# longfish/Multigrid-FEANet

Measured on AMD Instinct MI355X. Metric: DoF-updates/sec per V-cycle (fp64) + achieved HBM GB/s, 4097² Poisson, higher is better.
Workload: dtype f64; 1 GPU; 4097x4097 poisson f64 V-cycle, L=12, V(1,1) (MultiGrid.Step semantics), batch 1 per GPU; mode=single, batch=1, levels=12, parallelism=single GPU

## Files before the change

multigrid-feanet_amd/csrc/framed_ops.hip:

```cpp
#include "framed_strip.h"

namespace fea {

__device__ __forceinline__ int lin_block(int rev) {
  const int bid = xcd_remap(blockIdx.x, gridDim.x);
  return rev ? (int)gridDim.x - 1 - bid : bid;
}

__device__ __forceinline__ TaskId decode_task_lin(int nstrips, int ntr, int rev = 0) {
  const int per = ntr * nstrips;
  const int wpb = (per + kWaves - 1) / kWaves;
  const int bid = lin_block(rev);
  TaskId id;
  id.b = bid / wpb;
  const int w = (bid - id.b * wpb) * kWaves + __builtin_amdgcn_readfirstlane((int)(threadIdx.x >> 6));
  id.t = w / nstrips;
  id.s = w - id.t * nstrips;
  id.valid = w < per;
  return id;
}

template <typename T>
__device__ __forceinline__ void norm_partial(const MgArgs<T>& g, double ssq) {
  ssq = wave_sum(ssq);
// ... 1640 lines not shown
      if (y - 4 >= r0) iter(y - 4, std::integral_constant<int, 2 % D>{});
  }
}

template <typename T, bool MULTI>
__global__ __launch_bounds__(256) void k_mg_prolong2(MgArgs<T> g) {
  __shared__ T tab[MULTI ? FEA_MAX_PATTERNS * kTabStride : 1];
  __shared__ T ptb[MULTI ? FEA_MAX_PATTERNS * kTabStride : 1];
  if constexpr (MULTI) {
    load_tables<T>(tab, g.ktab, g.omd, g.ntab, ptb, g.ptab, g.nptab);
    __syncthreads();
  }
  const TaskId id = decode_task_lin(g.nstrips, g.ntr);
  if (!id.valid) return;
  if constexpr (sizeof(T) == 8) {
    if (id.t & 1) {
      prolong2_task<T, MULTI, true>(g, id, tab, ptb);
      return;
    }
  }
  prolong2_task<T, MULTI, false>(g, id, tab, ptb);
}

template <int SECOND, typename X>
__device__ __forceinline__ X& pick(X& a, X& b) {
  if constexpr (SECOND) return b;
  else return a;
}

#ifndef FEA_JOIN_AHEAD
#define FEA_JOIN_AHEAD 2
#endif
static_assert(FEA_JOIN_AHEAD == 2 || FEA_JOIN_AHEAD == 4, "join prefetch ring of 2 or 4 rows");
#ifndef FEA_JOIN_UNROLL
#define FEA_JOIN_UNROLL 4
#endif
constexpr int kJoinUnroll = FEA_JOIN_UNROLL;
static_assert(kJoinUnroll % FEA_JOIN_AHEAD == 0 && kJoinUnroll % 2 == 0, "join unroll: a multiple of the ring");
template <int N, typename Fn, int... I>
__device__ __forceinline__ void unroll_steps_(Fn&& fn, std::integer_sequence<int, I...>) {
  (fn(std::integral_constant<int, I>{}), ...);
}
template <int N, typename Fn>
__device__ __forceinline__ void unroll_steps(Fn&& fn) {
  unroll_steps_<N>(fn, std::make_integer_sequence<int, N>{});
}
// ... 850 lines not shown
template <typename T>
static int prolong2(const T* fc, const T* ec2, const T* f, T* out, const uint8_t* pid, const uint8_t* pidc,
                    const uint8_t* pidc2, const T* ktab, const T* omd, int ntab, const T* ptab, int nptab, T w1, int B,
                    int H, int W, int ld, long long bs, int ldc, long long bsc, int ldc2, long long bsc2,
                    void* stream) {
  if (!fc || !ec2 || !f || !out || !omd || !ptab || B <= 0 || !layout_ok<T>(H, W, ld, bs)) return FEA_EINVAL;
  if (!coarse_ok<T>(H, W, ldc, bsc) || !coarse_ok<T>((H + 1) / 2, (W + 1) / 2, ldc2, bsc2)) return FEA_EINVAL;
  const bool multi = ntab > 1;
  if (!tab_ok(ktab, ntab, pid) || (multi && (!pidc || !pidc2)) || !xtab_ok(nptab, ntab)) return FEA_EINVAL;
  MgArgs<T> g = mg_args<T>(H, W, ld, bs, B);
  g.ec = fc; g.ec2 = ec2; g.f = f; g.out = out; g.pid = pid; g.pidc = pidc; g.pidc2 = pidc2; g.ktab = ktab;
  g.omd = omd; g.ntab = ntab; g.ptab = ptab; g.nptab = nptab; g.w = w1;
  mg_coarse(g, ldc, bsc);
  mg_coarse2(g, ldc2, bsc2);
  g.nstrips = div_up(W - 2, Ovl4<T>::S);
  const int u2 = pick_rb(B, g.nstrips, H - 2) / 2;
  g.rb = 2 * balanced_units(B, g.nstrips, (H - 1) / 2, 2, 4, u2, u2);
  g.ntr = div_up(H - 2, g.rb);
  const dim3 grid = mg_grid_lin(B, g.ntr, g.nstrips);
  hipStream_t s = (hipStream_t)stream;
  if (multi) k_mg_prolong2<T, true><<<grid, 256, 0, s>>>(g);
  else k_mg_prolong2<T, false><<<grid, 256, 0, s>>>(g);
  return launch_status();
}

#define FEA_MG_API(SUF, T)                                                                                           \
  extern "C" int fea_mg_pack_##SUF(const T* src, T* dst, const T* geo, long long geo_bs, const T* bc, long long bc_bs, \
                                   int B, int H, int W, int ld, long long bs, void* stream) {                         \
    return mg_pack<T>(src, dst, geo, geo_bs, bc, bc_bs, B, H, W, ld, bs, stream);                                     \
  }                                                                                                                  \
  extern "C" int fea_mg_unpack_##SUF(const T* src, T* dst, int B, int H, int W, int ld, long long bs, void* stream) { \
    return mg_unpack<T>(src, dst, B, H, W, ld, bs, stream);                                                          \
  }                                                                                                                  \
  extern "C" int fea_mg_sweep_##SUF(const T* u, const T* f, T* out, const uint8_t* pid, const T* ktab, const T* omd,   \
                                    int ntab, int B, int H, int W, int ld, long long bs, void* stream) {              \
    return mg_sweep<T>(u, f, out, pid, ktab, omd, ntab, B, H, W, ld, bs, stream);                                    \
  }                                                                                                                  \
  extern "C" int fea_mg_residual_restrict_##SUF(const T* u, const T* f, T* v_out, T* fc, const uint8_t* pid,          \
                                                const T* ktab, const T* omd, int ntab, const T* rtab, int nrtab,      \
                                                T w0, int B, int H, int W, int ld, long long bs, int ldc,            \
                                                long long bsc, void* stream) {                                       \
    return mg_residual_restrict<T>(u, f, v_out, fc, pid, ktab, omd, ntab, rtab, nrtab, w0, B, H, W, ld, bs, ldc, bsc,  \
                                   stream);                                                                          \
  }                                                                                                                  \
  extern "C" int fea_mg_zero_restrict_send_##SUF(const T* f, T* fc, const uint8_t* pid, const T* ktab, const T* omd,   \
                                                 int ntab, const T* rtab, int nrtab, T w0, int B, int H, int W,       \
// ... 72 lines not shown
```

multigrid-feanet_amd/csrc/mid_ops.hip:

```cpp
#include "fea_common.h"

namespace fea {

constexpr int kMidThreads = 1024;
constexpr int kMidMaxK = 4;
constexpr int kMidLdsBytes = 160 * 1024 - 2048;
constexpr int kMS = 10;

#ifdef FEA_MID_TRACE
__device__ long long g_mid_trace[4096];
#define FEA_MID_MARK(slot) \
  if (threadIdx.x == 0) g_mid_trace[slot] = (long long)__builtin_amdgcn_s_memrealtime()
#define FEA_MID_SYNC(ph)                                                                   \
  do {                                                                                     \
    __syncthreads();                                                                       \
    if (blockIdx.x == 0 && threadIdx.x == 0) g_mid_trace[2048 + (ph)] = (long long)__builtin_amdgcn_s_memrealtime(); \
  } while (0)
#define FEA_MID_WAVE_MARK(slot)                                                              \
  if (blockIdx.x == 0 && (threadIdx.x & 63) == 0)                                            \
  g_mid_trace[3072 + (slot) * 16 + (threadIdx.x >> 6)] = (long long)__builtin_amdgcn_s_memrealtime()
#else
#define FEA_MID_MARK(slot)
#define FEA_MID_SYNC(ph) __syncthreads()
#define FEA_MID_WAVE_MARK(slot)
// ... 590 lines not shown
    const int Y0 = wv * per, Y1 = min(U0.nr, Y0 + per);
    constexpr int CH = MULTI ? 2 : 4;
    for (int s0 = Y0; s0 < Y1; s0 += CH) {
      const int n = min(CH, Y1 - s0);
      if constexpr (CH == 4) {
        if (n == 4) chunk(std::integral_constant<int, 4>{}, s0, s0 + 4);
        else if (n == 3) chunk(std::integral_constant<int, 3>{}, s0, s0 + 3);
        else if (n == 2) chunk(std::integral_constant<int, 2>{}, s0, s0 + 2);
        else chunk(std::integral_constant<int, 1>{}, s0, s0 + 1);
      } else {
        if (n == 2) chunk(std::integral_constant<int, 2>{}, s0, s0 + 2);
        else chunk(std::integral_constant<int, 1>{}, s0, s0 + 1);
      }
    }
    if (j > 0) FEA_MID_SYNC(1 + (k - 1 - j));
  }
  FEA_MID_MARK(2 * blockIdx.x + 1);
}

}

using namespace fea;

template <typename T>
static int mid_fill(MidArgs<T>& a, int k, int B, int H, int W, int TR, int TC) {
  if (k < 1 || k > kMidMaxK || B <= 0 || B > 65535 || TR < 1 || TC < 1) return FEA_EINVAL;
  a.k = k;
  for (int j = 0; j <= k; ++j) {
    if (H < 3 || W < 3 || (j < k && (!(H & 1) || !(W & 1)))) return FEA_EINVAL;
    a.H[j] = H;
    a.W[j] = W;
    if (fea_mg_layout(H, W, (int)sizeof(T), &a.ld[j], &a.bs[j]) != 0) return FEA_EINVAL;
    H = (H + 1) / 2;
    W = (W + 1) / 2;
  }
  a.TR = TR;
  a.TC = TC;
  return 0;
}

template <typename T, bool MULTI, typename Kern>
static void mid_launch(Kern k1, Kern k2, Kern k3, Kern k4, int k, dim3 grid, void* stream, const MidArgs<T>& a) {
  Kern kern = k == 1 ? k1 : k == 2 ? k2 : k == 3 ? k3 : k4;
  hipLaunchKernelGGL(kern, grid, dim3(kMidThreads), 0, (hipStream_t)stream, a);
}

template <typename T, bool GATHER>
static int mid_down(const T* const* f, const uint8_t* const* pid, int k, int B, int H, int W, const T* ktab,
                    const T* omd, int ntab, const T* rtab, int nrtab, T w0, int TR, int TC, const T* gsrc, int Pr,
                    int Pc, int gcr, int gcc, void* stream) {
  MidArgs<T> a = {};
  if (!f || !omd || !rtab || !tab_ok(ktab, ntab, pid) || !xtab_ok(nrtab, ntab)) return FEA_EINVAL;
  if (GATHER && (!gsrc || Pr < 1 || Pc < 1 || gcr < 1 || gcc < 1 || H - 1 != Pr * gcr || W - 1 != Pc * gcc))
    return FEA_EINVAL;
  const bool multi = ntab > 1;
  if (mid_fill<T>(a, k, B, H, W, TR, TC)) return FEA_EINVAL;
  if (mid_down_lds(k, TR, TC, (int)sizeof(T), multi) > kMidLdsBytes) return FEA_EINVAL;
  for (int j = 0; j <= k; ++j) {
    if (!f[j] || (multi && j < k && !pid[j])) return FEA_EINVAL;
    a.f[j] = f[j];
    a.fo[j] = const_cast<T*>(f[j]);
    a.pid[j] = multi && j < k ? pid[j] : nullptr;
  }
  a.ktab = ktab; a.omd = omd; a.xtab = rtab; a.w = w0; a.ntab = ntab; a.nx = nrtab;
  if (GATHER) {
    a.gsrc = gsrc; a.gB = B; a.gPc = Pc; a.gcr = gcr; a.gcc = gcc;
  }
  a.ntr = (a.H[k] - 2 + TR - 1) / TR;
  a.ntc = (a.W[k] - 2 + TC - 1) / TC;
  const dim3 grid(B * a.ntr * a.ntc);
  if (multi) mid_launch<T, true>(k_mg_mid_down<T, true, 1, GATHER>, k_mg_mid_down<T, true, 2, GATHER>,
                                 k_mg_mid_down<T, true, 3, GATHER>, k_mg_mid_down<T, true, 4, GATHER>, k, grid,
                                 stream, a);
  else mid_launch<T, false>(k_mg_mid_down<T, false, 1, GATHER>, k_mg_mid_down<T, false, 2, GATHER>,
                            k_mg_mid_down<T, false, 3, GATHER>, k_mg_mid_down<T, false, 4, GATHER>, k, grid,
                            stream, a);
  return launch_status();
}

template <typename T>
static int mid_up(const T* const* f, const T* e, T* out, const uint8_t* const* pid, int k, int B, int H, int W,
                  const T* ktab, const T* omd, int ntab, const T* ptab, int nptab, T w1, int TR, int TC,
                  void* stream) {
  MidArgs<T> a = {};
  if (!f || !e || !out || !omd || !ptab || !tab_ok(ktab, ntab, pid) || !xtab_ok(nptab, ntab)) return FEA_EINVAL;
  const bool multi = ntab > 1;
  if (mid_fill<T>(a, k, B, H, W, TR, TC)) return FEA_EINVAL;
  if (mid_up_lds(k, TR, TC, (int)sizeof(T), multi) > kMidLdsBytes) return FEA_EINVAL;
  for (int j = 0; j <= k; ++j) {
    if ((j < k && (!f[j] || f[j] == out)) || (multi && !pid[j])) return FEA_EINVAL;
    a.f[j] = j < k ? f[j] : nullptr;
    a.pid[j] = multi ? pid[j] : nullptr;
  }
  if (e == out) return FEA_EINVAL;
  a.e = e; a.out = out;
  a.ktab = ktab; a.omd = omd; a.xtab = ptab; a.w = w1; a.ntab = ntab; a.nx = nptab;
  a.ntr = (a.H[0] - 2 + TR - 1) / TR;
  a.ntc = (a.W[0] - 2 + TC - 1) / TC;
  const dim3 grid(B * a.ntr * a.ntc);
  if (multi) mid_launch<T, true>(k_mg_mid_up<T, true, 1>, k_mg_mid_up<T, true, 2>, k_mg_mid_up<T, true, 3>,
                                 k_mg_mid_up<T, true, 4>, k, grid, stream, a);
  else mid_launch<T, false>(k_mg_mid_up<T, false, 1>, k_mg_mid_up<T, false, 2>, k_mg_mid_up<T, false, 3>,
                            k_mg_mid_up<T, false, 4>, k, grid, stream, a);
  return launch_status();
}

#define FEA_MID_API(SUF, T)                                                                                        \
  extern "C" int fea_mg_mid_down_##SUF(const T* const* f, const uint8_t* const* pid, int k, int B, int H, int W,    \
                                       const T* ktab, const T* omd, int ntab, const T* rtab, int nrtab, T w0,       \
// ... 31 lines not shown
```

multigrid-feanet_amd/feanet_amd/schedule.py:

```python


def _other(b):
    return "b" if b == "a" else "a"


OMDF = "omdf"


def vcycle_schedule(L, nu1=1, nu2=1, compat=None, start="a", tail_from=None, fuse=True, top_zero=False,
                    recompute=True):
    if tail_from is not None and not (1 <= tail_from <= L - 1):
        raise ValueError("vcycle_schedule: tail_from must be in [1, L-1]")
    if L < 1 or nu1 < 0 or nu2 < 0:
        raise ValueError("vcycle_schedule: need L >= 1, nu1, nu2 >= 0")
    if compat not in (None, "mm_interface_q2"):
        raise ValueError(f"vcycle_schedule: unknown compat mode {compat!r}")
    steps = []
    cur = ["zero"] * L
    cur[0] = "zero" if top_zero else start

    def sweep(l, zero=False):
        dst = "a" if (zero or cur[l] == "zero") else _other(cur[l])
        steps.append(("sweep", l, None if (zero or cur[l] == "zero") else cur[l], dst))
        cur[l] = dst
# ... 174 lines not shown
            k = len(run)
            while k > 0:
                if k >= 2 and can_pair(run[k - 1][1]):
                    paired.append(("prolong_sweep2", run[k - 1][1], run[k - 2][3], run[k - 1][4]))
                    k -= 2
                else:
                    paired.append(run[k - 1])
                    k -= 1
            paired.reverse()
        else:
            k = 0
            while k < len(run):
                if k + 1 < len(run) and can_pair(run[k + 1][1]):
                    paired.append(("prolong_sweep2", run[k + 1][1], run[k][3], run[k + 1][4]))
                    k += 2
                else:
                    paired.append(run[k])
                    k += 1
        out.extend(paired)
        i = j
    return out


def group_mid(steps, pick_down, pick_up):
    out = []
    i = 0
    n = len(steps)
    while i < n:
        st = steps[i]
        if st[0] == "resid_restrict" and st[2] is None and st[3] is None:
            j = i
            while (j + 1 < n and steps[j + 1][0] == "resid_restrict" and steps[j + 1][2] is None
                   and steps[j + 1][3] is None and steps[j + 1][1] == steps[j][1] + 1):
                j += 1
            run = steps[i:j + 1]
            groups = {a: (k, T) for a, k, T in pick_down([s_[1] for s_ in run])}
            m = 0
            while m < len(run):
                l = run[m][1]
                if l in groups:
                    k, T = groups[l]
                    out.append(("mid_down", l, k, T))
                    m += k
                else:
                    out.append(run[m])
                    m += 1
# ... 44 lines not shown
```

multigrid-feanet_amd/feanet_amd/solver.py:

```python
import itertools
import math
import time
import weakref

import numpy as np
import torch

from . import _lib, mesh_setup as ms, ops
from .graphs import GraphCache
from .schedule import (OMDF, _other, extend_tail, group_hmid, group_mid, hjac_schedule, pair_prolongations, pair_restrictions,
                       vcycle_schedule)


_SOLVERS = weakref.WeakValueDictionary()
_HANDLES = itertools.count(1)


def first_sweep_raw(launches, f0, raw):
    for i, rec in enumerate(launches):
        try:
            _lib.arg(rec, "u_raw")
        except TypeError:
            continue
        if _lib.arg(rec, "f") == f0:
            return launches[:i] + [_lib.replace(rec, u_raw=raw)] + launches[i + 1:]
    return None


def solver_by_handle(h):
    s = _SOLVERS.get(int(h))
    if s is None:
        raise RuntimeError(f"feanet: no live MultigridSolver with handle {h}")
    return s
# ... 36 lines not shown
    def view(self, t):
        off = 128 // t.element_size() - 1
        return t[:self.B * self.bs].view(self.B, self.H + 2, self.ld)[:, 1:self.H + 1, off:off + self.W]

    def pid_view(self):
        return self.pid[:(self.H + 2) * self.ld].view(self.H + 2, self.ld)[1:self.H + 1, self.off:self.off + self.W]

    def geom(self):
        return (self.B, self.H, self.W, self.ld, self.bs)

    def geom_kw(self):
        return dict(B=self.B, H=self.H, W=self.W, ld=self.ld, bstride=self.bs)


class MultigridSolver:

    MID_NODES = 20000
    MID_NODES_DOWN = None
    MID_NODES_UP = None
    MID_MIN_TILES = 200
    MID_MAX_REDUNDANCY = 3.0
    HMID_NODES = 300000
    HMID_MIN_TILES = 64
    TAIL_MAX_N = 65
    TAIL_EXT = True
    TAIL_EXT_MIN_BATCH = 64

    def __init__(self, n, levels=None, problem="poisson", dtype=torch.float64, device=None, batch=1,
                 omega=2.0 / 3.0, size=2.0, prop=(1, 20), shape=0, R=None, P=None, w=(1.0, 1.0),
                 nu1=1, nu2=1, compat=None, graph=True, coarse_tail=True, fuse=True, rows=None, zero_start=False,
                 smoother="jac", hnet=None, join_cycles=True, mid=True, pair_levels=True, pid_maps=None):
        m = n if rows is None else int(rows)
        if rows is None and (n < 2 or (n & (n - 1)) != 0):
            raise ValueError(f"MultigridSolver: n={n} must be a power of two >= 2")
        if m < 2 or n < 2:
            raise ValueError(f"MultigridSolver: need >= 2 intervals each way (got {m} x {n})")
        if dtype not in (torch.float32, torch.float64):
            raise TypeError("MultigridSolver: dtype must be torch.float32 or torch.float64")
        self.device = torch.device(device if device is not None else "cuda")
        ops.require_hip(torch.empty(0, device=self.device), "solver device")
        self.n, self.m = n, m
        if levels is None:
            L = 1
            while (n % (1 << L) == 0 and m % (1 << L) == 0 and (n >> L) >= 2 and (m >> L) >= 2):
                L += 1
            self.L = L if rows is not None else int(math.log2(n))
# ... 235 lines not shown
            w = [float(x) for x in (w.detach().cpu().tolist() if torch.is_tensor(w) else w)]
            if (w[0], w[1]) != self.w:
                self.w = (w[0], w[1])
                self._plans.clear()
                self._graphs.clear()

    def _ptr(self, lvl, name):
        if name == OMDF:
            return None
        return self.levels[lvl].buf(name).data_ptr()

    def _build(self, start):
        if self.smoother == "hjac":
            steps, end = hjac_schedule(self.L, self.nu1, self.nu2, "zero" if self.zero_start else start,
                                       tail_from=self.hjac_tail_from, fuse=self.fuse)
            if self.mid and self.fuse:
                steps = group_hmid(steps, self._pick_hmid())
        else:
            steps, end = vcycle_schedule(self.L, self.nu1, self.nu2, self.compat, start, self.tail_from, self.fuse,
                                         top_zero=self.zero_start)
            if self.mid:
                steps = group_mid(steps, lambda lv: self._pick_mid(lv, False), lambda lv: self._pick_mid(lv, True))
            if self.pair_levels:
                ok = lambda l: l + 2 < self.L and self.levels[l + 2].H >= 3 and self.levels[l + 2].W >= 3
                steps = pair_prolongations(pair_restrictions(steps, ok), ok)
            if self._tail_ext_ok():
                steps = extend_tail(steps)
        return [self.bind_step(st) for st in steps], end

    def _tail_ext_ok(self):
        t = self.tail_from
        return (self.TAIL_EXT and t is not None and self.B >= self.TAIL_EXT_MIN_BATCH and self.ntab == 1
                and self.nu1 == 1 and self.nu2 == 1 and self.compat is None and self.levels[t - 1].W <= 129 and self.levels[t - 1].H <= 129)

    def _mid_tile(self, up, a, k):
        esz = self.levels[0].esz
        multi = self.ntab > 1
        tl = self.levels[a if up else a + k]
        top = self.levels[a]
        best = None
        for T in ((128, 64, 32, 16, 8) if up else (32, 16, 8, 4, 2)):
            if _lib.mid_lds_bytes(up, k, T, T, esz, multi) <= 0:
                continue
            tiles = self.B * -(-(tl.H - 2) // T) * -(-(tl.W - 2) // T)
            if not up:
                reg = (T << k) + 3 * ((1 << k) - 1)
                if reg * reg * tiles > self.MID_MAX_REDUNDANCY * self.B * top.H * top.W:
                    continue
            best = T
            if tiles >= self.MID_MIN_TILES:
                return T
# ... 84 lines not shown

        def fs(a, n):
            return _lib.PtrArray([lv[j].f.data_ptr() for j in range(a, a + n)])

        def tail(t):
            return dict(Ht=lv[t].H, Wt=lv[t].W, nlev=self.L - t, ld_t=lv[t].ld, bs_t=lv[t].bs,
                        pid_levels=None if self.tail_pid is None else self.tail_pid.data_ptr(),
                        ktab=self.ktab.data_ptr(), omd=self.omd.data_ptr(), ntab=self.ntab, rtab=self.rtab.data_ptr(),
                        ptab=self.ptab.data_ptr(), w0=self.w[0], w1=self.w[1], nu1=self.nu1, nu2=self.nu2, B=lv[t].B)

        kind, l = st[0], st[1]
        f = lv[l].f.data_ptr()
        if kind == "sweep":
            return launch("mg_sweep", u=ptr(l, st[2]), f=f, out=ptr(l, st[3]), **sten(pid(l)), **geom(l))
        if kind == "hsweep":
            return launch("mg_hsweep", u=ptr(l, st[2]), u_raw=None, f=f, out=ptr(l, st[3]), **sten(pid(l)),
                          **self._hnet(), **geom(l))
        if kind == "resid_restrict":
            return launch("mg_residual_restrict", u=ptr(l, st[2]), f=f, v_out=ptr(l, st[3]), fc=lv[l + 1].f.data_ptr(),
                          **sten(pid(l)), **rest(), **geom(l), **cp(l))
        if kind == "resid_restrict2":
            return launch("mg_zero_restrict2", f=f, fc=lv[l + 1].f.data_ptr(), fc2=lv[l + 2].f.data_ptr(),
                          pidc=pid(l + 1), **sten(pid(l)), **rest(), **geom(l), **cp(l), **cp2(l))
        if kind == "sweep_restrict":
            return launch("mg_sweep_restrict", u=ptr(l, st[2]), f=f, u_out=ptr(l, st[3]), fc=lv[l + 1].f.data_ptr(),
                          **sten(pid(l)), **rest(), **geom(l), **cp(l), norm_ws=None, norm_hist=None, norm_cnt=None)
        if kind == "prolong_sweep":
            return launch("mg_prolong_sweep", u=ptr(l, st[2]), ec=ptr(l + 1, st[3]), f=f, out=ptr(l, st[4]),
                          pidc=pid(l + 1), **sten(pid(l)), **prol(), **geom(l), **cp(l))
        if kind == "prolong_sweep2":
            return launch("mg_prolong2", fc=lv[l + 1].f.data_ptr(), ec2=ptr(l + 2, st[2]), f=f, out=ptr(l, st[3]),
                          pidc=pid(l + 1), pidc2=pid(l + 2), **sten(pid(l)), **prol(), **geom(l), **cp(l), **cp2(l))
        if kind == "prolong_add":
            return launch("mg_prolong_add", u=ptr(l, st[2]), ec=ptr(l + 1, st[3]), out=ptr(l, st[4]), pidc=pid(l + 1),
                          **prol(), **geom(l), **cp(l))
        if kind == "mid_down":
            a, k, T = st[1], st[2], st[3]
            TR, TC = T if isinstance(T, tuple) else (T, T)
            return launch("mg_mid_down", f=fs(a, k + 1), k=k, B=self.B, H=lv[a].H, W=lv[a].W,
                          **sten(pids(a, k + 1)), **rest(), TR=TR, TC=TC)
        if kind == "mid_up":
            a, k, csrc, dst, T = st[1:6]
            TR, TC = T if isinstance(T, tuple) else (T, T)
            return launch("mg_mid_up", f=fs(a, k), e=ptr(a + k, csrc), out=ptr(a, dst), k=k, B=self.B, H=lv[a].H,
                          W=lv[a].W, **sten(pids(a, k + 1)), **prol(), TR=TR, TC=TC)
        if kind == "coarse_tail":
# ... 424 lines not shown
```

Before: 129.0 billion DoF-updates/s.

## Fuse three coarse levels into single strip kernels for restriction and prolongation

Adds strip-based kernels that process three multigrid levels in one launch. One fuses zero-start residual and restriction over three levels, the other fuses prolongation with a Jacobi sweep across three levels. A schedule pass rewrites the steps just above the coarse tail into these kernels, with only the prolongation variant switched on by default. The aim is fewer launches and fewer round trips of intermediate coarse grids through HBM on the small upper-mid levels, at the cost of redundant halo work, higher register pressure and limited parallelism.

```diff
diff --git a/multigrid-feanet_amd/csrc/framed_ops.hip b/multigrid-feanet_amd/csrc/framed_ops.hip
--- a/multigrid-feanet_amd/csrc/framed_ops.hip
+++ b/multigrid-feanet_amd/csrc/framed_ops.hip
@@ -1686,6 +1686,521 @@
   prolong2_task<T, MULTI, false>(g, id, tab, ptb);
 }
 
+template <typename T>
+struct Mg3Args {
+  MgArgs<T> g;
+  T* out3;
+  const T* ec3;
+  int Hc3, Wc3, ldc3;
+  long long bsc3;
+};
+
+template <int SH, typename T>
+__device__ __forceinline__ T shrz(T x) {
+#pragma unroll
+  for (int k = 0; k < SH; ++k) x = shr1z(x);
+  return x;
+}
+template <int SH, typename T>
+__device__ __forceinline__ T shlz(T x) {
+#pragma unroll
+  for (int k = 0; k < SH; ++k) x = shl1z(x);
+  return x;
+}
+template <typename T, int N, int SH>
+__device__ __forceinline__ Row<T, N> own_row_sh(const T (&x)[N]) {
+  Row<T, N> w;
+#pragma unroll
+  for (int k = 0; k < N; ++k) w.a[k + 1] = x[k];
+  w.a[0] = shrz<SH>(x[N - 1]);
+  w.a[N + 1] = shlz<SH>(x[0]);
+  return w;
+}
+
+template <typename T, int N, int SH>
+struct RStage {
+  static constexpr int B0 = N == 1 ? 0 : 1;
+  Row<T, N> Va{}, Vb{}, Vc{};
+  Row<T, N> Ro{}, Re{};
+  T fp[N] = {};
+
+  template <bool ODD>
+  __device__ __forceinline__ T push(const T (&o)[N], bool rin, const bool (&jin)[N], const T (&ks)[9],
+                                    const T (&rs)[9], T om, T w0) {
+    T x[N];
+#pragma unroll
+    for (int q = 0; q < N; ++q) x[q] = (rin && jin[q]) ? om * o[q] : T(0);
+    Va = Vb;
+    Vb = Vc;
+    Vc = own_row_sh<T, N, SH>(x);
+    const PRow<N> np{};
+    T r[N];
+#pragma unroll
+    for (int q = 0; q < N; ++q) r[q] = fp[q] - kapply<T, N, false>(Va, Vb, Vc, np, np, np, q, ks, nullptr);
+    const Row<T, N> R = own_row_sh<T, N, SH>(r);
+    T out = T(0);
+    if constexpr (!ODD) {
+      const int zp[1] = {0};
+      const T acc = restrict9<T, false>(rs, nullptr, Ro.a, Re.a, R.a, B0, zp, zp, zp, 0);
+      out = w0 * acc;
+      Ro = R;
+    } else {
+      Re = R;
+    }
+#pragma unroll
+    for (int q = 0; q < N; ++q) fp[q] = o[q];
+    return out;
+  }
+};
+
+template <typename T>
+struct OvlZ3 {
+  static constexpr int V = Frame<T>::VEC;
+  static constexpr int Q = V / 2;
+  static constexpr int SH3 = Q == 1 ? 2 : 1;
+  static constexpr int LN = 2 * SH3;
+  static constexpr int L1 = 1, H1 = 62;
+  static constexpr int L2 = L1 + (Q == 1 ? 2 : 1), H2 = H1 - 2;
+  static constexpr int L3 = L2 + 2 * SH3, H3 = H2 - 2 * SH3;
+  static constexpr int I0 = L3;
+  static constexpr int NC = (H3 - I0) / LN + 1;
+  static constexpr int S = 8 * NC;
+  static_assert(I0 - SH3 >= L2 && I0 - (Q == 1 ? 3 : 1) >= L1 && I0 + LN * (NC - 1) <= H3, "owned lanes are exact");
+  static_assert(V * I0 + V - 1 - 8 <= Frame<T>::OFF, "the left halo fits the frame");
+};
+
+template <typename T>
+__global__ __launch_bounds__(256) void k_mg_zero_restrict3(Mg3Args<T> a) {
+  using F = Frame<T>;
+  using O = OvlZ3<T>;
+  constexpr int V = F::VEC;
+  constexpr int Q = O::Q;
+  const MgArgs<T>& g = a.g;
+  const TaskId id = decode_task_lin(g.nstrips, g.ntr);
+  if (!id.valid) return;
+  const int lane = lane_id();
+  const int H = g.H, W = g.W, Hc = g.Hc, Wc = g.Wc, Hc2 = g.Hc2, Wc2 = g.Wc2, Hc3 = a.Hc3, Wc3 = a.Wc3;
+  const int Nlo = id.s * O::NC + 1, Nhi = Nlo + O::NC;
+  const int Mlo = 2 * Nlo - 1, Mhi = 2 * Nhi - 1;
+  const int Jlo = 2 * Mlo - 1, Jhi = 2 * Mhi - 1;
+  const int cs = 8 * Nlo - (V - 1) - V * O::I0;
+  const int cl = cs + V * lane;
+  const int J0 = (cl + 1) / 2;
+  const int M0 = Q == 1 ? (J0 >> 1) : ((J0 + 1) >> 1);
+  const int N0 = M0 >> 1;
+  const bool has2 = Q == 1 ? !(J0 & 1) : true;
+  const bool has3 = has2 && !(M0 & 1);
+  const int K0 = 1 + id.t * (g.rb / 8);
+  const int K1 = min(K0 + g.rb / 8, Hc3 - 1);
+  const bool last = K1 == Hc3 - 1;
+  const int R2lo = 2 * K0 - 1, R2hi = last ? Hc2 - 1 : 2 * K1 - 1;
+  const int R1lo = 2 * R2lo - 1, R1hi = last ? Hc - 1 : 2 * R2hi - 1;
+  T ks[9], rs[9];
+#pragma unroll
+  for (int d = 0; d < 9; ++d) {
+    ks[d] = g.ktab[d];
+    rs[d] = g.rtab[d];
+  }
+  const T om = g.omd[0];
+  const T w0 = g.w;
+  bool cin[V], jin[Q], st1[Q];
+#pragma unroll
+  for (int k = 0; k < V; ++k) cin[k] = cl + k >= 1 && cl + k <= W - 2;
+#pragma unroll
+  for (int q = 0; q < Q; ++q) {
+    jin[q] = J0 + q >= 1 && J0 + q <= Wc - 2;
+    st1[q] = J0 + q >= Jlo && J0 + q < Jhi && J0 + q <= Wc - 2;
+  }
+  const bool min2[1] = {M0 >= 1 && M0 <= Wc2 - 2};
+  const bool st2 = has2 && M0 >= Mlo && M0 < Mhi && M0 <= Wc2 - 2;
+  const bool st3 = has3 && N0 >= Nlo && N0 < Nhi && N0 <= Wc3 - 2;
+  const T* __restrict__ fb = g.f + (long long)id.b * g.bs + F::OFF + cs;
+  T* __restrict__ cb = g.out + (long long)id.b * g.bsc + F::OFF + J0;
+  T* __restrict__ cb2 = g.out2 + (long long)id.b * g.bsc2 + F::OFF + M0;
+  T* __restrict__ cb3 = a.out3 + (long long)id.b * a.bsc3 + F::OFF + N0;
+  const int ld = g.ld;
+  const int ll = min(lane, (W - 1 - cs) / V);
+  auto rowo = [&](int r) -> long long { return (long long)(min(max(r, -1), H) + 1) * ld + V * ll; };
+
+  struct In {
+    T f[V];
+  };
+  struct Wn {
+    Row<T, V> v;
+    T f[V];
+  };
+  auto load = [&](int y) {
+    In r;
+    vload<T, V>(fb + rowo(y), r.f);
+    return r;
+  };
+  auto mk = [&](const In& r, int y) {
+    Wn w;
+    const bool rin = y >= 1 && y <= H - 2;
+    T x[V];
+#pragma unroll
+    for (int k = 0; k < V; ++k) {
+      x[k] = (rin && cin[k]) ? om * r.f[k] : T(0);
+      w.f[k] = r.f[k];
+    }
+    w.v = own_row<T, V>(x);
+    return w;
+  };
+  const PRow<V> np{};
+  const int zp[1] = {0};
+  auto resid = [&](const Wn& x0, const Wn& x1, const Wn& x2, T (&r)[V + 1]) {
+#pragma unroll
+    for (int k = 0; k < V; ++k) r[k] = x1.f[k] - kapply<T, V, false>(x0.v, x1.v, x2.v, np, np, np, k, ks, nullptr);
+    r[V] = shl1z(r[0]);
+  };
+
+  const int Ia = 4 * K0 - 6;
+  const In i0 = load(2 * Ia - 2), i1 = load(2 * Ia - 1), i2 = load(2 * Ia);
+  const In p0 = load(2 * Ia + 1), p1 = load(2 * Ia + 2);
+  In ring[4][2];
+#pragma unroll
+  for (int d = 0; d < 4; ++d) {
+    ring[d][0] = load(2 * (Ia + 1 + d) + 1);
+    ring[d][1] = load(2 * (Ia + 1 + d) + 2);
+  }
+  Wn X0 = mk(i0, 2 * Ia - 2), X1 = mk(i1, 2 * Ia - 1), X2 = mk(i2, 2 * Ia);
+  T Rp[V + 1], Rm[V + 1], Rn[V + 1];
+  resid(X0, X1, X2, Rp);
+  auto step = [&](const In& r, int y, T (&R)[V + 1]) {
+    X0 = X1;
+    X1 = X2;
+    X2 = mk(r, y);
+    resid(X0, X1, X2, R);
+  };
+  auto finish1 = [&](int I, T (&o)[Q]) {
+#pragma unroll
+    for (int q = 0; q < Q; ++q) {
+      const T acc = restrict9<T, false>(rs, nullptr, Rp, Rm, Rn, 2 * q, zp, zp, zp, 0);
+      o[q] = w0 * acc;
+    }
+    if (I >= R1lo && I < R1hi) {
+      T* cp = cb + (long long)(I + 1) * g.ldc;
+#pragma unroll
+      for (int q = 0; q < Q; ++q)
+        if (st1[q]) cp[q] = o[q];
+    }
+#pragma unroll
+    for (int k = 0; k <= V; ++k) Rp[k] = Rn[k];
+  };
+  auto row1 = [&](int I, auto slot, T (&o)[Q]) {
+    constexpr int SL = decltype(slot)::value;
+    step(ring[SL][0], 2 * I + 1, Rm);
+    ring[SL][0] = load(2 * I + 9);
+    step(ring[SL][1], 2 * I + 2, Rn);
+    ring[SL][1] = load(2 * I + 10);
+    finish1(I, o);
+  };
+  auto in1 = [&](int I) { return I >= 1 && I <= Hc - 2; };
+  auto in2 = [&](int Kr) { return Kr >= 1 && Kr <= Hc2 - 2; };
+
+  RStage<T, Q, 1> s2;
+  RStage<T, 1, O::SH3> s3;
+  auto row2 = [&](int Kr, T o2, auto odd_c) {
+    if (st2 && Kr >= R2lo && Kr < R2hi) cb2[(long long)(Kr + 1) * g.ldc2] = o2;
+    const T x[1] = {o2};
+    return s3.template push<decltype(odd_c)::value>(x, in2(Kr), min2, ks, rs, om, w0);
+  };
+  T o[Q];
+  step(p0, 2 * Ia + 1, Rm);
+  step(p1, 2 * Ia + 2, Rn);
+  finish1(Ia, o);
+  s2.template push<false>(o, in1(Ia), jin, ks, rs, om, w0);
+  int I = Ia + 1;
+  for (int K = K0 - 2; K < K1; ++K, I += 4) {
+    row1(I, std::integral_constant<int, 0>{}, o);
+    s2.template push<true>(o, in1(I), jin, ks, rs, om, w0);
+    row1(I + 1, std::integral_constant<int, 1>{}, o);
+    T o2 = s2.template push<false>(o, in1(I + 1), jin, ks, rs, om, w0);
+    row2(2 * K + 1, o2, std::true_type{});
+    row1(I + 2, std::integral_constant<int, 2>{}, o);
+    s2.template push<true>(o, in1(I + 2), jin, ks, rs, om, w0);
+    row1(I + 3, std::integral_constant<int, 3>{}, o);
+    o2 = s2.template push<false>(o, in1(I + 3), jin, ks, rs, om, w0);
+    const T o3 = row2(2 * K + 2, o2, std::false_type{});
+    if (st3 && K >= K0) cb3[(long long)(K + 1) * a.ldc3] = o3;
+  }
+}
+
+template <typename T>
+struct OvlP3 {
+  static constexpr int V = Frame<T>::VEC;
+  static constexpr int SH2 = V == 2 ? 2 : 1;
+  static constexpr int LO = SH2 + 3, HI = 63 - 2 * SH2 - 2;
+  static constexpr int S = (HI - LO + 1) * V;
+  static_assert(LO * V - 1 <= Frame<T>::OFF, "the left halo fits the frame");
+};
+
+template <typename T>
+__global__ __launch_bounds__(256) void k_mg_prolong3(Mg3Args<T> a) {
+  using F = Frame<T>;
+  using O = OvlP3<T>;
+  constexpr int V = F::VEC;
+  constexpr int Q = V / 2;
+  constexpr int SH2 = O::SH2;
+  const MgArgs<T>& g = a.g;
+  const TaskId id = decode_task_lin(g.nstrips, g.ntr);
+  if (!id.valid) return;
+  const int lane = lane_id();
+  const int H = g.H, Hc = g.Hc, W = g.W, Wc = g.Wc, Hc2 = g.Hc2, Wc2 = g.Wc2, Hc3 = a.Hc3, Wc3 = a.Wc3;
+  const int c0 = 1 + id.s * O::S;
+  const int cs = c0 - O::LO * V;
+  const int cl = cs + V * lane;
+  const int r0 = 1 + id.t * g.rb;
+  const int r1 = min(r0 + g.rb, H - 1);
+  T ks[9], ps[9];
+#pragma unroll
+  for (int d = 0; d < 9; ++d) {
+    ks[d] = g.ktab[d];
+    ps[d] = g.ptab[d];
+  }
+  const T om = g.omd[0];
+  const T w1 = g.w;
+  const int ld = g.ld, ldc = g.ldc, ldc2 = g.ldc2, ldc3 = a.ldc3;
+  bool cin[V];
+#pragma unroll
+  for (int k = 0; k < V; ++k) cin[k] = cl + k >= 1 && cl + k <= W - 2;
+  const bool own = lane >= O::LO && lane <= O::HI;
+  const int ll = min(lane, (W - 1 - cs) / V);
+  const long long boff = (long long)id.b * g.bs + F::OFF + cs;
+  const T* __restrict__ fb = g.f + boff;
+  T* __restrict__ ob = g.out + boff;
+  const int jc = (cs + 1) / 2;
+  const int J0 = jc + Q * lane;
+  const int KL = (J0 - 1) >> 1;
+  bool jin[Q];
+#pragma unroll
+  for (int q = 0; q < Q; ++q) jin[q] = J0 + q >= 1 && J0 + q <= Wc - 2;
+  const bool kin = KL >= 1 && KL <= Wc2 - 2;
+  const T* __restrict__ f2b = g.ec + (long long)id.b * g.bsc + F::OFF + jc + Q * ll;
+  const T* __restrict__ f3b = g.ec2 + (long long)id.b * g.bsc2 + F::OFF + min(max(KL, 0), Wc2 - 1);
+  const T* __restrict__ e4b = a.ec3 + (long long)id.b * a.bsc3 + F::OFF + min(max((KL - 1) >> 1, -1), Wc3 - 2);
+  auto rowo = [&](int r) -> long long { return (long long)(min(max(r, -1), H) + 1) * ld + V * ll; };
+  auto crowo = [&](int r) -> long long { return (long long)(min(max(r, -1), Hc) + 1) * ldc; };
+  auto c2rowo = [&](int r) -> long long { return (long long)(min(max(r, -1), Hc2) + 1) * ldc2; };
+  auto c3rowo = [&](int r) -> long long { return (long long)(min(max(r, -1), Hc3) + 1) * ldc3; };
+  const PRow<1> np1{};
+  const PRow<Q> npq{};
+  const PRow<V> npv{};
+
+  auto pterm = [&](const T (&e)[2], int col, int ky) -> T {
+    if (col & 1) {
+      T t = ps[ky * 3 + 2] * e[0];
+      t += ps[ky * 3 + 0] * e[1];
+      return t;
+    }
+    return ps[ky * 3 + 1] * e[1];
+  };
+
+  struct In3 {
+    T f;
+    T e[2][2];
+  };
+  auto ld3 = [&](int d) {
+    In3 r;
+    r.f = f3b[c2rowo(d)];
+#pragma unroll
+    for (int h = 0; h < 2; ++h) {
+      const long long o = c3rowo((d >> 1) + h);
+      r.e[h][0] = e4b[o];
+      r.e[h][1] = e4b[o + 1];
+    }
+    return r;
+  };
+  struct X3 {
+    Row<T, 1> x;
+    T f;
+  };
+  auto mkx3 = [&](const In3& r, int d) {
+    const bool din = d >= 1 && d <= Hc2 - 2;
+    T x[1];
+    x[0] = (din && kin) ? om * r.f : T(0);
+    if (d & 1) {
+      const T t = pterm(r.e[0], KL, 2) + pterm(r.e[1], KL, 0);
+      x[0] += w1 * t;
+    } else {
+      x[0] += w1 * pterm(r.e[0], KL, 1);
+    }
+    X3 w;
+    w.x = own_row_sh<T, 1, SH2>(x);
+    w.f = r.f;
+    return w;
+  };
+  struct E2 {
+    T e[2];
+  };
+  auto mku3 = [&](const X3& x0, const X3& x1, const X3& x2, int c) {
+    const bool cin3 = c >= 1 && c <= Hc2 - 2;
+    const T u = jacobi<T, 1, false>(x0.x, x1.x, x2.x, np1, np1, np1, 0, x1.f, ks, om, nullptr);
+    E2 r;
+    r.e[0] = (cin3 && kin) ? u : T(0);
+    r.e[1] = shlz<SH2>(r.e[0]);
+    return r;
+  };
+
+  struct In2 {
+    T f[Q];
+  };
+  auto ld2 = [&](int b) {
+    In2 r;
+    vload<T, Q>(f2b + crowo(b), r.f);
+    return r;
+  };
+  struct X2 {
+    Row<T, Q> x;
+    T f[Q];
+  };
+  auto mkx2 = [&](const In2& r, int b, const E2& lo, const E2& hi) {
+    const bool bin = b >= 1 && b <= Hc - 2;
+    T x[Q];
+#pragma unroll
+    for (int q = 0; q < Q; ++q) x[q] = (bin && jin[q]) ? om * r.f[q] : T(0);
+#pragma unroll
+    for (int q = 0; q < Q; ++q) {
+      const int Jq = J0 + q;
+      if (b & 1) {
+        const T t = pterm(lo.e, Jq, 2) + pterm(hi.e, Jq, 0);
+        x[q] += w1 * t;
+      } else {
+        x[q] += w1 * pterm(lo.e, Jq, 1);
+      }
+    }
+    X2 w;
+    w.x = own_row<T, Q>(x);
+#pragma unroll
+    for (int q = 0; q < Q; ++q) w.f[q] = r.f[q];
+    return w;
+  };
+  auto mku2 = [&](const X2& a_, const X2& b_, const X2& c_, int r) {
+    const bool ain = r >= 1 && r <= Hc - 2;
+    T o[Q];
+#pragma unroll
+    for (int q = 0; q < Q; ++q) {
+      const T u = jacobi<T, Q, false>(a_.x, b_.x, c_.x, npq, npq, npq, q, b_.f[q], ks, om, nullptr);
+      o[q] = (ain && jin[q]) ? u : T(0);
+    }
+    CRow<T, V> c{};
+#pragma unroll
+    for (int q = 0; q < Q; ++q) c.e[q + 1] = o[q];
+    c.e[0] = shr1z(o[Q - 1]);
+    return c;
+  };
+
+  struct In {
+    T f[V];
+  };
+  struct XR {
+    Row<T, V> x;
+    T f[V];
+  };
+  auto ld_f = [&](int y) {
+    In r;
+    vload<T, V>(fb + rowo(y), r.f);
+    return r;
+  };
+  auto zero_iterate = [&](const In& r, int y, T (&x)[V]) {
+    const bool rin = y >= 1 && y <= H - 2;
+#pragma unroll
+    for (int k = 0; k < V; ++k) x[k] = (rin && cin[k]) ? om * r.f[k] : T(0);
+  };
+  auto finish_x = [&](const In& r, const T (&x)[V]) {
+    XR w;
+    w.x = own_row<T, V>(x);
+#pragma unroll
+    for (int k = 0; k < V; ++k) w.f[k] = r.f[k];
+    return w;
+  };
+  auto row_even = [&](const In& r, int y, const CRow<T, V>& ca) {
+    T x[V];
+    zero_iterate(r, y, x);
+#pragma unroll
+    for (int k = 0; k < V; ++k) x[k] += w1 * crow_term<T, V, false>(ca, k + 1, 1, ps, nullptr);
+    return finish_x(r, x);
+  };
+  auto row_odd = [&](const In& r, int y, const CRow<T, V>& ca, const CRow<T, V>& cb) {
+    T x[V];
+    zero_iterate(r, y, x);
+#pragma unroll
+    for (int k = 0; k < V; ++k) {
+      const T t = crow_term<T, V, false>(ca, k + 1, 2, ps, nullptr) + crow_term<T, V, false>(cb, k + 1, 0, ps, nullptr);
+      x[k] += w1 * t;
+    }
+    return finish_x(r, x);
+  };
+  auto emit = [&](int y, const XR& xa, const XR& xb, const XR& xc) {
+    T o[V];
+#pragma unroll
+    for (int k = 0; k < V; ++k) {
+      o[k] = jacobi<T, V, false>(xa.x, xb.x, xc.x, npv, npv, npv, k, xb.f[k], ks, om, nullptr);
+    }
+    if (own && y < r1) store_masked<T, V, false>(ob + rowo(y), o, cl, W);
+  };
+
+  const int a0 = (r0 - 1) / 2;
+  const int cq = a0 / 2;
+  const In3 t0 = ld3(cq - 2), t1 = ld3(cq - 1), t2 = ld3(cq), t3 = ld3(cq + 1), t4 = ld3(cq + 2);
+  In3 n3 = ld3(cq + 3);
+  const In2 s0 = ld2(a0 - 1), s1 = ld2(a0), s2 = ld2(a0 + 1), s3 = ld2(a0 + 2);
+  const In f0 = ld_f(r0 - 1), f1 = ld_f(r0);
+  struct Slot {
+    In u1, u2;
+    In2 c;
+  };
+  Slot ring[2];
+  auto fill = [&](Slot& sl, int y) {
+    sl.u1 = ld_f(y + 1);
+    sl.u2 = ld_f(y + 2);
+    sl.c = ld2((y + 5) / 2);
+  };
+  fill(ring[0], r0);
+  fill(ring[1], r0 + 2);
+  X3 Ya = mkx3(t0, cq - 2), Yb = mkx3(t1, cq - 1), Yc = mkx3(t2, cq);
+  const E2 Um = mku3(Ya, Yb, Yc, cq - 1);
+  Ya = Yb, Yb = Yc, Yc = mkx3(t3, cq + 1);
+  E2 U0 = mku3(Ya, Yb, Yc, cq);
+  Ya = Yb, Yb = Yc, Yc = mkx3(t4, cq + 2);
+  E2 U1 = mku3(Ya, Yb, Yc, cq + 1);
+  X2 Xa = mkx2(s0, a0 - 1, Um, U0);
+  X2 Xb = mkx2(s1, a0, U0, U0);
+  X2 Xc2 = mkx2(s2, a0 + 1, U0, U1);
+  const CRow<T, V> C0 = mku2(Xa, Xb, Xc2, a0);
+  Xa = Xb, Xb = Xc2, Xc2 = mkx2(s3, a0 + 2, U1, U1);
+  CRow<T, V> C1 = mku2(Xa, Xb, Xc2, a0 + 1);
+  XR Xp = row_even(f0, r0 - 1, C0);
+  XR Xc = row_odd(f1, r0, C0, C1);
+  auto iter = [&](int y, auto slot, int dn) {
+    constexpr int SL = decltype(slot)::value;
+    Slot& sl = ring[SL];
+    if constexpr (SL == 0) {
+      Ya = Yb, Yb = Yc, Yc = mkx3(n3, dn);
+      n3 = ld3(dn + 1);
+      U0 = U1;
+      U1 = mku3(Ya, Yb, Yc, dn - 1);
+    }
+    const XR Xn = row_even(sl.u1, y + 1, C1);
+    emit(y, Xp, Xc, Xn);
+    Xa = Xb, Xb = Xc2;
+    if constexpr (SL == 0) Xc2 = mkx2(sl.c, (y + 5) / 2, U0, U1);
+    else Xc2 = mkx2(sl.c, (y + 5) / 2, U1, U1);
+    const CRow<T, V> C2 = mku2(Xa, Xb, Xc2, (y + 3) / 2);
+    const XR Xnn = row_odd(sl.u2, y + 2, C1, C2);
+    emit(y + 1, Xc, Xn, Xnn);
+    Xp = Xn;
+    Xc = Xnn;
+    C1 = C2;
+    fill(sl, y + 4);
+  };
+  int dn = cq + 3;
+  for (int y = r0; y < r1; y += 4, ++dn) {
+    iter(y, std::integral_constant<int, 0>{}, dn);
+    iter(y + 2, std::integral_constant<int, 1>{}, dn);
+  }
+}
+
 template <int SECOND, typename X>
 __device__ __forceinline__ X& pick(X& a, X& b) {
   if constexpr (SECOND) return b;
@@ -2582,6 +3097,82 @@
   if (multi) k_mg_prolong2<T, true><<<grid, 256, 0, s>>>(g);
   else k_mg_prolong2<T, false><<<grid, 256, 0, s>>>(g);
   return launch_status();
+}
+
+template <typename T>
+static bool mg_coarse3(Mg3Args<T>& a, int ldc2, long long bsc2, int ldc3, long long bsc3) {
+  MgArgs<T>& g = a.g;
+  if (!coarse_ok<T>(g.Hc, g.Wc, ldc2, bsc2)) return false;
+  mg_coarse2(g, ldc2, bsc2);
+  if (!coarse_ok<T>(g.Hc2, g.Wc2, ldc3, bsc3)) return false;
+  a.Hc3 = (g.Hc2 + 1) / 2; a.Wc3 = (g.Wc2 + 1) / 2; a.ldc3 = ldc3; a.bsc3 = bsc3;
+  return true;
+}
+
+template <typename T>
+static int zero_restrict3(const T* f, T* fc, T* fc2, T* fc3, const uint8_t* pid, const T* ktab, const T* omd, int ntab,
+                          const T* rtab, int nrtab, T w0, int B, int H, int W, int ld, long long bs, int ldc,
+                          long long bsc, int ldc2, long long bsc2, int ldc3, long long bsc3, int units, void* stream) {
+  if (!restrict_ok<T>(f, fc, pid, ktab, ntab, rtab, nrtab, B, H, W, ld, bs, ldc, bsc) || !fc2 || !fc3 || !omd ||
+      ntab != 1 || units < 0)
+    return FEA_EINVAL;
+  Mg3Args<T> a{};
+  MgArgs<T>& g = a.g;
+  g = mg_args<T>(H, W, ld, bs, B);
+  g.f = f; g.out = fc; g.out2 = fc2; a.out3 = fc3; g.pid = pid; g.ktab = ktab; g.omd = omd; g.ntab = ntab;
+  g.rtab = rtab; g.nrtab = nrtab; g.w = w0;
+  mg_coarse(g, ldc, bsc);
+  if (!mg_coarse3(a, ldc2, bsc2, ldc3, bsc3)) return FEA_EINVAL;
+  g.nstrips = div_up(W - 2, OvlZ3<T>::S);
+  const int rows_u = a.Hc3 - 2;
+  const int u = units > 0 ? std::min(units, rows_u) : balanced_units(B, g.nstrips, rows_u, 8, 21, 1);
+  g.rb = 8 * u;
+  g.ntr = div_up(rows_u, u);
+  k_mg_zero_restrict3<T><<<mg_grid_lin(B, g.ntr, g.nstrips), 256, 0, (hipStream_t)stream>>>(a);
+  return launch_status();
+}
+
+template <typename T>
+static int prolong3(const T* fc, const T* fc2, const T* ec3, const T* f, T* out, const uint8_t* pid, const T* ktab,
+                    const T* omd, int ntab, const T* ptab, int nptab, T w1, int B, int H, int W, int ld, long long bs,
+                    int ldc, long long bsc, int ldc2, long long bsc2, int ldc3, long long bsc3, int units,
+                    void* stream) {
+  if (!fc || !fc2 || !ec3 || !f || !out || !omd || !ptab || B <= 0 || !layout_ok<T>(H, W, ld, bs)) return FEA_EINVAL;
+  if (!coarse_ok<T>(H, W, ldc, bsc) || !tab_ok(ktab, ntab, pid) || !xtab_ok(nptab, ntab) || ntab != 1 || units < 0)
+    return FEA_EINVAL;
+  Mg3Args<T> a{};
+  MgArgs<T>& g = a.g;
+  g = mg_args<T>(H, W, ld, bs, B);
+  g.ec = fc; g.ec2 = fc2; a.ec3 = ec3; g.f = f; g.out = out; g.pid = pid; g.ktab = ktab; g.omd = omd; g.ntab = ntab;
+  g.ptab = ptab; g.nptab = nptab; g.w = w1;
+  mg_coarse(g, ldc, bsc);
+  if (!mg_coarse3(a, ldc2, bsc2, ldc3, bsc3)) return FEA_EINVAL;
+  g.nstrips = div_up(W - 2, OvlP3<T>::S);
+  const int rows_u = div_up(H - 2, 4);
+  const int u = units > 0 ? std::min(units, rows_u) : balanced_units(B, g.nstrips, rows_u, 4, 10, 1);
+  g.rb = 4 * u;
+  g.ntr = div_up(H - 2, g.rb);
+  k_mg_prolong3<T><<<mg_grid_lin(B, g.ntr, g.nstrips), 256, 0, (hipStream_t)stream>>>(a);
+  return launch_status();
+}
+
+namespace fea {
+#define FEA_STRIP3(T)                                                                                                \
+  int strip_zero_restrict3(const T* f, T* fc, T* fc2, T* fc3, const T* ktab, const T* omd, int ntab, const T* rtab,  \
+                           int nrtab, T w0, int B, int H, int W, const int* ld, const long long* bs, int units,      \
+                           void* stream) {                                                                           \
+    return zero_restrict3<T>(f, fc, fc2, fc3, nullptr, ktab, omd, ntab, rtab, nrtab, w0, B, H, W, ld[0], bs[0],      \
+                             ld[1], bs[1], ld[2], bs[2], ld[3], bs[3], units, stream);                               \
+  }                                                                                                                  \
+  int strip_prolong3(const T* fc, const T* fc2, const T* ec3, const T* f, T* out, const T* ktab, const T* omd,       \
+                     int ntab, const T* ptab, int nptab, T w1, int B, int H, int W, const int* ld,                   \
+                     const long long* bs, int units, void* stream) {                                                 \
+    return prolong3<T>(fc, fc2, ec3, f, out, nullptr, ktab, omd, ntab, ptab, nptab, w1, B, H, W, ld[0], bs[0],       \
+                       ld[1], bs[1], ld[2], bs[2], ld[3], bs[3], units, stream);                                     \
+  }
+FEA_STRIP3(float)
+FEA_STRIP3(double)
+#undef FEA_STRIP3
 }
 
 #define FEA_MG_API(SUF, T)                                                                                           \
diff --git a/multigrid-feanet_amd/csrc/mid_ops.hip b/multigrid-feanet_amd/csrc/mid_ops.hip
--- a/multigrid-feanet_amd/csrc/mid_ops.hip
+++ b/multigrid-feanet_amd/csrc/mid_ops.hip
@@ -636,6 +636,30 @@
 
 using namespace fea;
 
+namespace fea {
+#define FEA_STRIP3_DECL(T)                                                                                          \
+  int strip_zero_restrict3(const T* f, T* fc, T* fc2, T* fc3, const T* ktab, const T* omd, int ntab, const T* rtab, \
+                           int nrtab, T w0, int B, int H, int W, const int* ld, const long long* bs, int units,     \
+                           void* stream);                                                                           \
+  int strip_prolong3(const T* fc, const T* fc2, const T* ec3, const T* f, T* out, const T* ktab, const T* omd,      \
+                     int ntab, const T* ptab, int nptab, T w1, int B, int H, int W, const int* ld,                  \
+                     const long long* bs, int units, void* stream);
+FEA_STRIP3_DECL(float)
+FEA_STRIP3_DECL(double)
+#undef FEA_STRIP3_DECL
+}
+static inline bool mid_strips(int TR, int TC) { return TR < 0 && TC == -1; }
+
+template <typename T>
+static bool strip_layouts(int H, int W, int (&ld)[4], long long (&bs)[4]) {
+  for (int j = 0; j < 4; ++j) {
+    if (fea_mg_layout(H, W, (int)sizeof(T), &ld[j], &bs[j]) != 0) return false;
+    H = (H + 1) / 2;
+    W = (W + 1) / 2;
+  }
+  return true;
+}
+
 template <typename T>
 static int mid_fill(MidArgs<T>& a, int k, int B, int H, int W, int TR, int TC) {
   if (k < 1 || k > kMidMaxK || B <= 0 || B > 65535 || TR < 1 || TC < 1) return FEA_EINVAL;
@@ -668,6 +692,14 @@
   if (GATHER && (!gsrc || Pr < 1 || Pc < 1 || gcr < 1 || gcc < 1 || H - 1 != Pr * gcr || W - 1 != Pc * gcc))
     return FEA_EINVAL;
   const bool multi = ntab > 1;
+  if (!GATHER && mid_strips(TR, TC)) {
+    int ld[4];
+    long long bs[4];
+    if (k != 3 || multi || B > 65535 || !strip_layouts<T>(H, W, ld, bs) || !f[0] || !f[1] || !f[2] || !f[3])
+      return FEA_EINVAL;
+    return strip_zero_restrict3(f[0], const_cast<T*>(f[1]), const_cast<T*>(f[2]), const_cast<T*>(f[3]), ktab, omd,
+                                ntab, rtab, nrtab, w0, B, H, W, ld, bs, -TR, stream);
+  }
   if (mid_fill<T>(a, k, B, H, W, TR, TC)) return FEA_EINVAL;
   if (mid_down_lds(k, TR, TC, (int)sizeof(T), multi) > kMidLdsBytes) return FEA_EINVAL;
   for (int j = 0; j <= k; ++j) {
@@ -699,6 +731,14 @@
   MidArgs<T> a = {};
   if (!f || !e || !out || !omd || !ptab || !tab_ok(ktab, ntab, pid) || !xtab_ok(nptab, ntab)) return FEA_EINVAL;
   const bool multi = ntab > 1;
+  if (mid_strips(TR, TC)) {
+    int ld[4];
+    long long bs[4];
+    if (k != 3 || multi || B > 65535 || !strip_layouts<T>(H, W, ld, bs) || !f[0] || !f[1] || !f[2] || e == out ||
+        f[0] == out || f[1] == out || f[2] == out)
+      return FEA_EINVAL;
+    return strip_prolong3(f[1], f[2], e, f[0], out, ktab, omd, ntab, ptab, nptab, w1, B, H, W, ld, bs, -TR, stream);
+  }
   if (mid_fill<T>(a, k, B, H, W, TR, TC)) return FEA_EINVAL;
   if (mid_up_lds(k, TR, TC, (int)sizeof(T), multi) > kMidLdsBytes) return FEA_EINVAL;
   for (int j = 0; j <= k; ++j) {
diff --git a/multigrid-feanet_amd/feanet_amd/schedule.py b/multigrid-feanet_amd/feanet_amd/schedule.py
--- a/multigrid-feanet_amd/feanet_amd/schedule.py
+++ b/multigrid-feanet_amd/feanet_amd/schedule.py
@@ -220,6 +220,31 @@
     return out
 
 
+def group_triples(steps, can_down, can_up):
+    zr = lambda st: st[0] == "resid_restrict" and st[2] is None and st[3] is None
+    ps = lambda st: st[0] == "prolong_sweep" and st[2] == OMDF
+    out = list(steps)
+    for i, st in enumerate(steps):
+        if st[0] != "coarse_tail":
+            continue
+        t, c = st[1], st[2]
+        lo = i
+        while lo > 0 and zr(steps[lo - 1]) and steps[lo - 1][1] == t - (i - lo) - 1:
+            lo -= 1
+        hi = i + 1
+        src = c
+        while hi < len(steps) and ps(steps[hi]) and steps[hi][1] == t - (hi - i) and steps[hi][3] == src:
+            src = steps[hi][4]
+            hi += 1
+        nd, nu = i - lo, hi - i - 1
+        if nu >= 3 and nu % 2 == 1 and can_up(t - 3):
+            out[i + 1:i + 4] = [("prolong_sweep3", t - 3, c, steps[i + 3][4])]
+        if nd >= 3 and nd % 2 == 1 and can_down(t - 3):
+            out[i - 3:i] = [("resid_restrict3", t - 3)]
+        break
+    return out
+
+
 def group_mid(steps, pick_down, pick_up):
     out = []
     i = 0
diff --git a/multigrid-feanet_amd/feanet_amd/solver.py b/multigrid-feanet_amd/feanet_amd/solver.py
--- a/multigrid-feanet_amd/feanet_amd/solver.py
+++ b/multigrid-feanet_amd/feanet_amd/solver.py
@@ -8,7 +8,7 @@
 
 from . import _lib, mesh_setup as ms, ops
 from .graphs import GraphCache
-from .schedule import (OMDF, _other, extend_tail, group_hmid, group_mid, hjac_schedule, pair_prolongations, pair_restrictions,
+from .schedule import (OMDF, _other, extend_tail, group_hmid, group_mid, group_triples, hjac_schedule, pair_prolongations, pair_restrictions,
                        vcycle_schedule)
 
 
@@ -91,6 +91,10 @@
     MID_MAX_REDUNDANCY = 3.0
     HMID_NODES = 300000
     HMID_MIN_TILES = 64
+    THREE_LEVEL_UP = True
+    THREE_LEVEL_DOWN = False
+    STRIP2_COLUMNS = {8: 116, 4: 244}
+    BAL2_WAVES = 1024
     TAIL_MAX_N = 65
     TAIL_EXT = True
     TAIL_EXT_MIN_BATCH = 64
@@ -372,11 +376,22 @@
             if self.mid:
                 steps = group_mid(steps, lambda lv: self._pick_mid(lv, False), lambda lv: self._pick_mid(lv, True))
             if self.pair_levels:
+                if self.mid:
+                    steps = group_triples(steps, lambda l: self.THREE_LEVEL_DOWN and self._three_level_ok(l),
+                                          lambda l: self.THREE_LEVEL_UP and self._three_level_ok(l))
                 ok = lambda l: l + 2 < self.L and self.levels[l + 2].H >= 3 and self.levels[l + 2].W >= 3
                 steps = pair_prolongations(pair_restrictions(steps, ok), ok)
             if self._tail_ext_ok():
                 steps = extend_tail(steps)
         return [self.bind_step(st) for st in steps], end
+
+    def _three_level_ok(self, l):
+        top = self.levels[l]
+        strips = -(-(top.W - 2) // self.STRIP2_COLUMNS[top.esz])
+        launch_bound = self.B * strips * max(((top.H + 1) // 2 + 1) // 2 - 2, 1) < self.BAL2_WAVES
+        return (self.smoother == "jac" and self.ntab == 1 and self.nu1 == 1 and self.nu2 == 1 and self.compat is None
+                and not self.zero_start and self.tail_from is not None and l >= 1 and l + 3 == self.tail_from
+                and not self._tail_ext_ok() and launch_bound)
 
     def _tail_ext_ok(self):
         t = self.tail_from
@@ -507,6 +522,12 @@
         if kind == "resid_restrict2":
             return launch("mg_zero_restrict2", f=f, fc=lv[l + 1].f.data_ptr(), fc2=lv[l + 2].f.data_ptr(),
                           pidc=pid(l + 1), **sten(pid(l)), **rest(), **geom(l), **cp(l), **cp2(l))
+        if kind == "resid_restrict3":
+            return launch("mg_mid_down", f=fs(l, 4), k=3, B=self.B, H=lv[l].H, W=lv[l].W, **sten(pids(l, 4)),
+                          **rest(), TR=-1, TC=-1)
+        if kind == "prolong_sweep3":
+            return launch("mg_mid_up", f=fs(l, 3), e=ptr(l + 3, st[2]), out=ptr(l, st[3]), k=3, B=self.B, H=lv[l].H,
+                          W=lv[l].W, **sten(pids(l, 4)), **prol(), TR=-1, TC=-1)
         if kind == "sweep_restrict":
             return launch("mg_sweep_restrict", u=ptr(l, st[2]), f=f, u_out=ptr(l, st[3]), fc=lv[l + 1].f.data_ptr(),
                           **sten(pid(l)), **rest(), **geom(l), **cp(l), norm_ws=None, norm_hist=None, norm_cnt=None)
```

Result: faster. 131.5 billion DoF-updates/s, median of 6 (+1.9%).
